# makezur/super_primitive

Hardware: AMD Instinct MI355X
Metric: GN iters/sec (640x480x64-seg frame pairs) (higher is better)
Workload: dtype f32; 1 GPU; Replica-shaped two-frame SfM, 640x480, 64 segments (grid, 4 px overlap), pyramid level 0 of a 3-level pyramid; BASELINE.json configs[1]; pairs_per_gpu=384, segment_pixels_per_pair=373056, optimiser=gn, tile_points=8192, span_points=4096, granule=64

## Files before the change

### super_primitive_amd/csrc/sp_cost.hip

```cpp
#include <type_traits>

#include "sp_solve_device.h"

namespace {

struct TileCtx {
    gptr_u32 pix;
    gptr_f4 src4;
    gptr_f32 trg;
    Cam Ks;
    Warp w;
    float shift;
    float gain, bias;
    float ax, ay;
    uint32_t row_bytes;
    int Wl, Hl;
    int start, count;
};

struct Geo {
    float qx, qy, qz;
    float zinv, zi;
    float px, py, pz;
};
// ... 194 lines not shown
    asm("v_pk_add_f32 %0, %1, %2 neg_lo:[0,1] neg_hi:[0,1]" : "=v"(d) : "v"(a), "v"(b));
    return d;
}
__device__ __forceinline__ f32x2 pmul_hi(f32x2 a, f32x2 b) {
    f32x2 d;
    asm("v_pk_mul_f32 %0, %1, %2 op_sel:[1,0] op_sel_hi:[1,1]" : "=v"(d) : "v"(a), "v"(b));
    return d;
}
__device__ __forceinline__ f32x2 pfma_lo(f32x2 a, f32x2 b, f32x2 c) {
    f32x2 d;
    asm("v_pk_fma_f32 %0, %1, %2, %3 op_sel:[0,0,0] op_sel_hi:[0,1,1]" : "=v"(d) : "v"(a), "v"(b), "v"(c));
    return d;
}
__device__ __forceinline__ f32x2 pfnma_lo(f32x2 a, f32x2 b, f32x2 c) {
    f32x2 d;
    asm("v_pk_fma_f32 %0, %1, %2, %3 op_sel:[0,0,0] op_sel_hi:[0,1,1] neg_lo:[1,0,0] neg_hi:[1,0,0]" : "=v"(d) : "v"(a), "v"(b), "v"(c));
    return d;
}
__device__ __forceinline__ f32x2 pfnma_hi(f32x2 a, f32x2 b, f32x2 c) {
    f32x2 d;
    asm("v_pk_fma_f32 %0, %1, %2, %3 op_sel:[1,0,0] op_sel_hi:[1,1,1] neg_lo:[1,0,0] neg_hi:[1,0,0]" : "=v"(d) : "v"(a), "v"(b), "v"(c));
    return d;
}
__device__ __forceinline__ f32x2 pfma_swz_lo(f32x2 a, f32x2 b, f32x2 c) {
    f32x2 d;
    asm("v_pk_fma_f32 %0, %1, %2, %3 op_sel:[1,0,0] op_sel_hi:[0,0,1]" : "=v"(d) : "v"(a), "v"(b), "v"(c));
    return d;
}
__device__ __forceinline__ f32x2 pfma_swz_hi(f32x2 a, f32x2 b, f32x2 c) {
    f32x2 d;
    asm("v_pk_fma_f32 %0, %1, %2, %3 op_sel:[1,1,0] op_sel_hi:[0,1,1]" : "=v"(d) : "v"(a), "v"(b), "v"(c));
    return d;
}
__device__ __forceinline__ f32x2 pmul_lo(f32x2 a, f32x2 b) {
    f32x2 d;
    asm("v_pk_mul_f32 %0, %1, %2 op_sel:[0,0] op_sel_hi:[0,1]" : "=v"(d) : "v"(a), "v"(b));
    return d;
}
__device__ __forceinline__ f32x2 pfma(float a, f32x2 b, f32x2 c) { return __builtin_elementwise_fma(f32x2{a, a}, b, c); }

struct GnAcc {
    f32x2 h00;
    f32x2 h0[2];
    f32x2 h1[2];
    f32x2 blk[6];
    f32x2 bp01;
    f32x2 bp[2];
    f32x2 hd01;
    f32x2 hd[2];
    float h11;
    f32x2 D, bd;
    float cost, n;
    float cost_mark, n_mark;
};

struct Pending2 {
    f32x2 qxy; float qz, zinv, zi;
    f32x2 wxy; float m;
    f32x2 srg; float sb;
    uint32_t off0;
};

__device__ __forceinline__ void prepare2_at(const PairConsts& k, f32x2 colrow, bool src_ok, float d, const f32x4 s, Pending2& p);

template <bool DT = false>
__device__ __forceinline__ void prepare2(const TileCtx& c, const PairConsts& k, float shift, uint32_t pw, const f32x4 s, Pending2& p) {
    const f32x2 colrow{(float)(pw & 0xffffu), (float)((pw >> 16) & 0x7fffu)};
    const bool src_ok = (int32_t)pw < 0;
    const float d = DT ? s.w * shift : fast_exp(s.w + shift);
    prepare2_at(k, colrow, src_ok, d, s, p);
}

typedef const SpRunDesc __attribute__((address_space(4)))* cptr_rd;
__device__ __forceinline__ SpRunDesc rd_load(cptr_rd p) {
    SpRunDesc r;
    r.valid[0] = p->valid[0]; r.valid[1] = p->valid[1];
    r.d[0] = p->d[0]; r.d[1] = p->d[1];
    r.base[0] = p->base[0]; r.base[1] = p->base[1];
    r.k = p->k; r.runs = p->runs;
    return r;
}
__device__ __forceinline__ f32x2 rd_colrow(const SpRunDesc& r, f32x2 lane2) {
    const float step = __builtin_amdgcn_fmed3f(lane2.x + r.k, 0.f, 1.f);
    return pfma(step, f32x2{r.d[0], r.d[1]}, lane2) + f32x2{r.base[0], r.base[1]};
}
__device__ __forceinline__ float rd_depth(const SpRunDesc& r, float d) {
    const uint64_t m = ((uint64_t)r.valid[1] << 32) | r.valid[0];
    float o;
    asm("v_cndmask_b32_e64 %0, 0, %1, %2" : "=v"(o) : "v"(d), "s"(m));
    return o;
}
template <bool DT>
__device__ __forceinline__ void prepare2_rd(const PairConsts& k, float shift, const SpRunDesc& r, f32x2 lane2, const f32x4 s, Pending2& p) {
    const f32x2 colrow = rd_colrow(r, lane2);
    const float d = rd_depth(r, DT ? s.w * shift : fast_exp(s.w + shift));
    prepare2_at(k, colrow, true, d, s, p);
}
template <bool DT>
__device__ __forceinline__ void prepare_rd(const TileCtx& c, float shift, float ifx, float ify, const SpRunDesc& r, f32x2 lane2, const f32x4 s,
                                           Pending& p) {
    const f32x2 colrow = rd_colrow(r, lane2);
    const float d = rd_depth(r, DT ? s.w * shift : fast_exp(s.w + shift));
    float x, y;
    backproject(colrow.x, colrow.y, d, c.Ks, ifx, ify, x, y);
    prepare_xyz(c, x, y, d, true, s.x, s.y, s.z, p);
}

__device__ __forceinline__ void prepare2_at(const PairConsts& k, f32x2 colrow, bool src_ok, float d, const f32x4 s, Pending2& p) {
    const f32x2 xy = pfma(colrow, k.ifxy, k.nKc) * d;
    const f32x2 qxy = pfma(k.R03, f32x2{xy.x, xy.x}, pfma(k.R14, f32x2{xy.y, xy.y}, pfma(k.R25, f32x2{d, d}, k.t01)));
    const float qz = fmaf(k.R6, xy.x, fmaf(k.R7, xy.y, fmaf(k.R8, d, k.t2)));
    const bool zguard = fabsf(qz) > 1e-6f;
    const float zinv = zguard ? __builtin_amdgcn_rcpf(qz) : 1e-6f;
    const f32x2 uv = qxy * k.Kf * zinv + k.Ktc;
    const f32x2 n = pfma(uv, k.invWH, f32x2{-1.f, -1.f});
    const bool ok = (fabsf(n.x) <= 0.99f) && (fabsf(n.y) <= 0.99f) && (qz > k.zmin) && src_ok && (d > 1e-7f);
    p.m = ok ? 1.f : 0.f;
    p.qxy = qxy; p.qz = qz;
    p.zinv = ok ? zinv : 0.f;
    p.zi = (ok && zguard) ? zinv : 0.f;
    p.srg = f32x2{s.x, s.y}; p.sb = s.z;
    const f32x2 ixy = pfma(n, k.sxy, k.sxy);
    const f32x2 fl{floorf(ixy.x), floorf(ixy.y)};
    p.wxy = ixy - fl;
    p.off0 = (uint32_t)fmaf(fl.y, k.row_bytes_f, fl.x * (float)(4u * SP_TEXEL_FLOATS));
}

struct Mix2 { f32x2 wa, wb, v; };
struct MixA { f32x2 ua, ub; };
struct AffAcc {
    float haa, hab, hbb, ba, bb;
    f32x2 pa01, pa[2], pb01, pb[2];
    float hda, hdb;
};

template <bool AFF = false>
__device__ __forceinline__ void finish_gn2(const PairConsts& k, const Pending2& p, const f32x3 a, const f32x3 b,
                                           const f32x3 cc, const f32x3 d, Mix2& o, float& cost_acc, float& n_acc,
                                           MixA* oa = nullptr, AffAcc* aa = nullptr) {
    const float eps = k.eps;
    const f32x2 a2{a.x, a.y}, b2{b.x, b.y}, c2{cc.x, cc.y}, d2{d.x, d.y};
    const f32x2 e3 = padd2(psub2(psub2(d2, c2), b2), a2);
    const f32x2 Er{b.x - a.x, cc.x - a.x}, Eg{b.y - a.y, cc.y - a.y}, Eb{b.z - a.z, cc.z - a.z};
    f32x2 e3b;
    e3b.x = (d.z - cc.z) - Eb.x;
    const f32x2 Gr = pfma_swz_lo(p.wxy, e3, Er), Gg = pfma_swz_hi(p.wxy, e3, Eg), Gb = pfma_swz_lo(p.wxy, e3b, Eb);
    const f32x2 it2{fmaf(p.wxy.y, Gr.y, fmaf(p.wxy.x, Er.x, a.x)), fmaf(p.wxy.y, Gg.y, fmaf(p.wxy.x, Eg.x, a.y))};
    const float itb = fmaf(p.wxy.y, Gb.y, fmaf(p.wxy.x, Eb.x, a.z));
    const f32x2 r2 = p.srg - pfma(k.gain, it2, k.bias2);
    const float rb = p.sb - fmaf(k.gain, itb, k.bias2.x);
    const float ar0 = fabsf(r2.x), ar1 = fabsf(r2.y), arb = fabsf(rb);
    auto absmax = [&](float r) { float m; asm("v_max_f32 %0, |%1|, %2" : "=v"(m) : "v"(r), "s"(eps)); return m; };
    const f32x2 wg2{__builtin_amdgcn_rcpf(absmax(r2.x)), __builtin_amdgcn_rcpf(absmax(r2.y))};
    const float wgb = __builtin_amdgcn_rcpf(absmax(rb));
    const f32x2 wGr = pmul_lo(wg2, Gr), wGg = pmul_hi(wg2, Gg), wGb = Gb * wgb;
    o.wa = pfma_lo(wGb, Gb, pfma_lo(wGg, Gg, pmul_lo(wGr, Gr)));
    o.wb = pfma_hi(wGb, Gb, pfma_hi(wGg, Gg, pmul_hi(wGr, Gr)));
    o.v = pfma(wGb, rb, pfma_hi(r2, wGg, pmul_lo(r2, wGr)));
    cost_acc = fmaf(p.m, (ar0 + ar1) + arb, cost_acc);
    n_acc += p.m;
    if constexpr (AFF) {
        const f32x2 ja2 = k.gain * it2;
        const float jab = k.gain * itb;
        const f32x2 wj2 = wg2 * ja2;
        const float wjb = wgb * jab;
        aa->haa = fmaf(p.m, fmaf(wjb, jab, wj2.x * ja2.x) + wj2.y * ja2.y, aa->haa);
        aa->hab = fmaf(-p.m, (wj2.x + wj2.y) + wjb, aa->hab);
        aa->hbb = fmaf(p.m, (wg2.x + wg2.y) + wgb, aa->hbb);
        aa->ba = fmaf(p.m, fmaf(wjb, rb, wj2.x * r2.x) + wj2.y * r2.y, aa->ba);
        aa->bb = fmaf(-p.m, fmaf(wgb, rb, wg2.x * r2.x) + wg2.y * r2.y, aa->bb);
        oa->ua = pfma(Gb, wjb, pfma_hi(wj2, Gg, pmul_lo(wj2, Gr)));
        oa->ub = (wGr + wGg) + wGb;
    }
}

struct GeoGn { f32x2 qxy; float qz, zinv, zi; };
template <bool AFF = false>
__device__ __forceinline__ void fold_gn2(const PairConsts& k, const GeoGn g, const Mix2 w, GnAcc& A, const MixA* wa = nullptr,
                                         AffAcc* aa = nullptr) {
    const f32x2 g2 = k.gab * g.zinv;
    const f32x2 Wa = w.wa * pmul_lo(g2, g2);
    const f32x2 Wb = w.wb * pmul_hi(g2, g2);
    const f32x2 V = -(w.v * g2);
    const f32x2 qxy = g.qxy;
    const f32x2 u = qxy * g.zi;
    const float ez = g.qz - k.t2;
    const f32x2 Q = pfma(-ez, u, qxy - k.t01);
    float nqy;
    asm("v_xor_b32 %0, 0x80000000, %1" : "=v"(nqy) : "v"(qxy.y));
    const f32x2 nA00{u.x, u.x * qxy.y}, A01{fmaf(u.x, qxy.x, g.qz), nqy};
    const f32x2 nA10{u.y, fmaf(u.y, qxy.y, g.qz)}, A11{u.y * qxy.x, qxy.x};
    const f32x2 nB00 = pfma_lo(Wa, nA00, pmul_hi(Wa, nA10)), B01 = pfma_lo(Wa, A01, pmul_hi(Wa, A11));
    const f32x2 nB10 = pfma_lo(Wb, nA00, pmul_hi(Wb, nA10)), B11 = pfma_lo(Wb, A01, pmul_hi(Wb, A11));
    const f32x2 P = pfma_lo(Q, Wa, pmul_hi(Q, Wb));
    A.h00 += Wa; A.h11 += Wb.y;
    A.h0[0] -= nB00; A.h0[1] += B01;
    A.h1[0] -= nB10; A.h1[1] += B11;
    A.blk[0] = pfma_lo(nA00, nB00, pfma_lo(nA10, nB10, A.blk[0]));
    A.blk[1] = pfnma_lo(nA00, B01, pfnma_lo(nA10, B11, A.blk[1]));
    A.blk[2] = pfma_hi(nA00, nB00, pfma_hi(nA10, nB10, A.blk[2]));
    A.blk[3] = pfnma_hi(nA00, B01, pfnma_hi(nA10, B11, A.blk[3]));
    A.blk[4] = pfma_lo(A01, B01, pfma_lo(A11, B11, A.blk[4]));
    A.blk[5] = pfma_hi(A01, B01, pfma_hi(A11, B11, A.blk[5]));
    A.bp01 += V;
    A.hd01 += P;
    A.bp[0] = pfnma_lo(V, nA00, pfnma_hi(V, nA10, A.bp[0]));
    A.bp[1] = pfma_lo(V, A01, pfma_hi(V, A11, A.bp[1]));
    A.hd[0] = pfnma_lo(P, nA00, pfnma_hi(P, nA10, A.hd[0]));
    A.hd[1] = pfma_lo(P, A01, pfma_hi(P, A11, A.hd[1]));
    A.D = pfma(Q, P, A.D);
    A.bd = pfma(Q, V, A.bd);
    if constexpr (AFF) {
        const f32x2 Ua = -(wa->ua * g2), Ub = wa->ub * g2;
        aa->pa01 += Ua;
        aa->pa[0] = pfnma_lo(Ua, nA00, pfnma_hi(Ua, nA10, aa->pa[0]));
        aa->pa[1] = pfma_lo(Ua, A01, pfma_hi(Ua, A11, aa->pa[1]));
        aa->hda = fmaf(Q.x, Ua.x, fmaf(Q.y, Ua.y, aa->hda));
        aa->pb01 += Ub;
        aa->pb[0] = pfnma_lo(Ub, nA00, pfnma_hi(Ub, nA10, aa->pb[0]));
        aa->pb[1] = pfma_lo(Ub, A01, pfma_hi(Ub, A11, aa->pb[1]));
        aa->hdb = fmaf(Q.x, Ub.x, fmaf(Q.y, Ub.y, aa->hdb));
    }
}

typedef const float __attribute__((address_space(4)))* cptr_f32;
struct ChunkRec { int pair, seg, start, count; };
typedef const ChunkRec __attribute__((address_space(4)))* cptr_i4;

struct SpanCursor {
    cptr_i4 chunks;
    cptr_f32 kld, kp_L;
    int q, q_end;
    int left;
    float shift;
    int nq_left;
    float nq_kld, nq_kpl;
};

template <int TRIP = SP_BLOCK>
__device__ __forceinline__ void cursor_fetch_next(SpanCursor& k) {
    if (k.q + 1 < k.q_end) {
        const int seg = k.chunks[k.q + 1].seg;
        k.nq_left = k.chunks[k.q + 1].count / TRIP;
        k.nq_kld = k.kld[seg];
        k.nq_kpl = k.kp_L[seg];
    }
}

template <bool DT>
__device__ __forceinline__ float cursor_shift(float kld, float kpl) { return DT ? fast_exp(kld - kpl) : kld - kpl; }

template <int TRIP = SP_BLOCK, bool DT = false>
__device__ __forceinline__ void cursor_init(SpanCursor& k, const SpPair& pr, const int4* chunks, int q0, int n) {
    k.chunks = (cptr_i4)chunks;
    k.kld = (cptr_f32)pr.kld;
    k.kp_L = (cptr_f32)pr.kp_L;
    k.q = q0; k.q_end = q0 + n;
    const int seg0 = k.chunks[q0].seg;
    k.left = k.chunks[q0].count / TRIP;
    k.shift = cursor_shift<DT>(k.kld[seg0], k.kp_L[seg0]);
    k.nq_left = 0; k.nq_kld = 0.f; k.nq_kpl = 0.f;
    cursor_fetch_next<TRIP>(k);
}

template <int TRIP = SP_BLOCK, bool DT = false>
__device__ __forceinline__ bool cursor_advance(SpanCursor& k, int& done_q) {
    done_q = k.q;
    if (--k.left > 0) return false;
    ++k.q;
    k.left = k.nq_left;
    k.shift = cursor_shift<DT>(k.nq_kld, k.nq_kpl);
    cursor_fetch_next<TRIP>(k);
    return true;
}

template <bool WT>
__device__ __forceinline__ void store_partial(float* p, float v) {
    if (WT) __hip_atomic_store(p, v, __ATOMIC_RELAXED, __HIP_MEMORY_SCOPE_AGENT);
    else *p = v;
}

__device__ __forceinline__ int lane_id() { return (int)__builtin_amdgcn_mbcnt_hi(~0u, __builtin_amdgcn_mbcnt_lo(~0u, 0u)); }

template <bool WT, bool AFF = false>
__device__ __forceinline__ void flush_segment_gn(GnAcc& A, float* __restrict__ rec, AffAcc* aa = nullptr) {
    const int lane = lane_id();
    int pos; bool ok;
    if constexpr (AFF) {
        float v[10] = {A.hd01.x, A.hd01.y, A.hd[0].x, A.hd[0].y, A.hd[1].x, A.hd[1].y, A.D.x + A.D.y, A.bd.x + A.bd.y, aa->hda, aa->hdb};
        wave_sum_to_lanes<10>(v, lane, pos, ok);
        if (ok) store_partial<WT>(rec + pos, v[0]);
        aa->hda = 0.f; aa->hdb = 0.f;
    } else {
        float v[10] = {A.hd01.x, A.hd01.y, A.hd[0].x, A.hd[0].y, A.hd[1].x, A.hd[1].y, A.D.x + A.D.y, A.bd.x + A.bd.y,
                       A.cost - A.cost_mark, A.n - A.n_mark};
        wave_sum_to_lanes<10>(v, lane, pos, ok);
        if (ok) store_partial<WT>(rec + pos, v[0]);
        A.cost_mark = A.cost; A.n_mark = A.n;
    }
    const f32x2 z{0.f, 0.f};
    A.hd01 = z; A.hd[0] = z; A.hd[1] = z; A.D = z; A.bd = z;
}

template <bool DT, bool WT, bool AFF = false, bool W64 = false, bool RD = false>
__device__ __forceinline__ void run_span_gn(const TileCtx& c, const SpPair& pr, const int4* __restrict__ chunks, int q0,
                                            int n_chunks, int total, float irls_eps, float* __restrict__ span_rec,
                                            float* __restrict__ seg_partials, float* lds, const SpRunDesc* rd = nullptr) {
    static_assert(!RD || (W64 && DT && !AFF), "run descriptors: wave spans on depth tables");
    constexpr int TRIP = W64 ? 64 : SP_BLOCK;
    constexpr int NV = AFF ? SP_GNA_PARTIAL_FLOATS : SP_GN_PARTIAL_FLOATS, NS = AFF ? SP_GNA_SEG_FLOATS : SP_GN_SEG_FLOATS;
    GnAcc A;
    AffAcc AA;
    MixA ma{f32x2{0.f, 0.f}, f32x2{0.f, 0.f}};
    {
        const f32x2 z{0.f, 0.f};
        AA.haa = AA.hab = AA.hbb = AA.ba = AA.bb = AA.hda = AA.hdb = 0.f;
        AA.pa01 = z; AA.pb01 = z; AA.pa[0] = z; AA.pa[1] = z; AA.pb[0] = z; AA.pb[1] = z;
    }
    {
        const f32x2 z{0.f, 0.f};
        A.h00 = z; A.bp01 = z; A.hd01 = z;
#pragma unroll
        for (int k = 0; k < 2; ++k) { A.h0[k] = z; A.h1[k] = z; A.bp[k] = z; A.hd[k] = z; }
#pragma unroll
        for (int k = 0; k < 6; ++k) A.blk[k] = z;
        A.D = z; A.bd = z;
        A.h11 = A.cost = A.n = A.cost_mark = A.n_mark = 0.f;
    }
    const int wave = __builtin_amdgcn_readfirstlane((int)(threadIdx.x >> 6));
    SpanCursor k;
    cursor_init<TRIP, DT>(k, pr, chunks, q0, n_chunks);
    const int start = k.chunks[q0].start;
    PairConsts kc;
    {
        const Warp& w = c.w;
        kc.ifxy = sgpr2(1.f / c.Ks.fx, 1.f / c.Ks.fy);
        kc.nKc = f32x2{-c.Ks.cx * (1.f / c.Ks.fx), -c.Ks.cy * (1.f / c.Ks.fy)};
        kc.R03 = sgpr2(w.R[0], w.R[3]);        kc.R14 = sgpr2(w.R[1], w.R[4]);      kc.R25 = sgpr2(w.R[2], w.R[5]);
        kc.t01 = f32x2{w.t[0], w.t[1]};        kc.Kf = sgpr2(w.Kt.fx, w.Kt.fy);     kc.Ktc = sgpr2(w.Kt.cx, w.Kt.cy);
        kc.invWH = sgpr2(2.f * w.invWm1, 2.f * w.invHm1);  kc.sxy = sgpr2(w.sx, w.sy);
        kc.gab = sgpr2(c.gain * c.ax * w.Kt.fx, c.gain * c.ay * w.Kt.fy);
        kc.bias2 = f32x2{c.bias, c.bias};      kc.eps2 = sgpr2(irls_eps, irls_eps);
        kc.R6 = sgpr(w.R[6]); kc.R7 = sgpr(w.R[7]); kc.R8 = sgpr(w.R[8]); kc.t2 = w.t[2];
        asm volatile("" : "+v"(kc.nKc), "+v"(kc.bias2), "+v"(kc.t01), "+v"(kc.t2));
        kc.gain = sgpr(c.gain); kc.bias = sgpr(c.bias); kc.zmin = sgpr(w.zmin); kc.eps = sgpr(irls_eps);
        kc.row_bytes_f = sgpr((float)(c.Wl * (int)(4u * SP_TEXEL_FLOATS)));
    }
    const rsrc_t r_pix = make_rsrc(c.pix + start, (uint32_t)total * 4u);
    const rsrc_t r_src = make_rsrc(c.src4 + start, (uint32_t)total * 16u);
    const rsrc_t r_trg = make_rsrc(c.trg, (uint32_t)c.Wl * (uint32_t)c.Hl * (4u * SP_TEXEL_FLOATS));
    const int n_iter = total / TRIP;
    uint32_t op = (W64 ? (threadIdx.x & 63u) : threadIdx.x) * 4u;
    constexpr int NT = 2;
    cptr_rd rg = (cptr_rd)rd + (start >> 6);
    f32x2 lane2{(float)(threadIdx.x & 63u), 0.f};
    if (RD) asm volatile("" : "+v"(lane2));
    struct Slot { Pending2 p; int q; bool last; };
    Slot S0, S1;
    {
        const f32x4 s = buf_load4<NT>(r_src, op * 4u);
        if (RD) prepare2_rd<DT>(kc, k.shift, rd_load(rg), lane2, s, S0.p);
        else {
            const uint32_t pw = (uint32_t)__builtin_amdgcn_raw_buffer_load_b32(r_pix, (int)op, 0, NT);
            prepare2<DT>(c, kc, k.shift, pw, s, S0.p);
        }
        S0.last = cursor_advance<TRIP, DT>(k, S0.q);
    }
    S1.p = S0.p;
    S1.p.zinv = 0.f; S1.p.zi = 0.f;
    S1.q = q0; S1.last = false;
    Mix2 m{f32x2{0.f, 0.f}, f32x2{0.f, 0.f}, f32x2{0.f, 0.f}};
    auto trip = [&](Slot& a, Slot& b) {
        op += 4u * TRIP;
        asm volatile("" : "+v"(op));
        const uint32_t pw = RD ? 0u : (uint32_t)__builtin_amdgcn_raw_buffer_load_b32(r_pix, (int)op, 0, NT);
        const f32x4 s = buf_load4<NT>(r_src, op * 4u);
        SpRunDesc rn;
        if (RD) { ++rg; rn = rd_load(rg); }
        f32x3 ta = buf_load3(r_trg, a.p.off0);
        f32x3 tb = buf_load3(r_trg, a.p.off0 + 4u * SP_TEXEL_FLOATS);
        f32x3 tc = buf_load3(r_trg, a.p.off0, c.row_bytes);
        f32x3 td = buf_load3(r_trg, a.p.off0 + 4u * SP_TEXEL_FLOATS, c.row_bytes);
        __builtin_amdgcn_sched_barrier(0);
        fold_gn2<AFF>(kc, GeoGn{b.p.qxy, b.p.qz, b.p.zinv, b.p.zi}, m, A, &ma, &AA);
        if (b.last) flush_segment_gn<WT, AFF>(A, seg_partials + (size_t)(W64 ? b.q : 4 * b.q + wave) * NS, &AA);
        __builtin_amdgcn_sched_barrier(0);
        asm volatile("" : "+v"(ta), "+v"(tb), "+v"(tc), "+v"(td), "+v"(A.blk[0]), "+v"(A.blk[1]), "+v"(A.blk[2]),
                     "+v"(A.blk[3]), "+v"(A.blk[4]), "+v"(A.blk[5]), "+v"(A.bp[0]), "+v"(A.bp[1]), "+v"(A.hd[0]),
                     "+v"(A.hd[1]), "+v"(A.D), "+v"(A.bd), "+v"(A.h00), "+v"(A.h0[0]), "+v"(A.h0[1]), "+v"(A.h1[0]), "+v"(A.h1[1]), "+v"(A.h11), "+v"(A.bp01), "+v"(A.hd01));
        finish_gn2<AFF>(kc, a.p, ta, tb, tc, td, m, A.cost, A.n, &ma, &AA);
        uint32_t pw_ = pw;
        f32x4 s_ = s;
        if (RD) asm volatile("" : "+v"(s_));
        else asm volatile("" : "+v"(pw_), "+v"(s_));
        if (RD) prepare2_rd<DT>(kc, k.shift, rn, lane2, s_, b.p);
        else prepare2<DT>(c, kc, k.shift, pw_, s_, b.p);
        b.last = cursor_advance<TRIP, DT>(k, b.q);
    };
    int j = 0;
    for (; j + 1 < n_iter; j += 2) { trip(S0, S1); trip(S1, S0); }
    if (j < n_iter) {
        trip(S0, S1);
        fold_gn2<AFF>(kc, GeoGn{S0.p.qxy, S0.p.qz, S0.p.zinv, S0.p.zi}, m, A, &ma, &AA);
        flush_segment_gn<WT, AFF>(A, seg_partials + (size_t)(W64 ? S0.q : 4 * S0.q + wave) * NS, &AA);
    } else {
        fold_gn2<AFF>(kc, GeoGn{S1.p.qxy, S1.p.qz, S1.p.zinv, S1.p.zi}, m, A, &ma, &AA);
        flush_segment_gn<WT, AFF>(A, seg_partials + (size_t)(W64 ? S1.q : 4 * S1.q + wave) * NS, &AA);
    }
    float acc[NV];
    acc[0] = A.cost;
    acc[1] = A.h00.x; acc[2] = A.h00.y;
    acc[3] = A.h0[0].x; acc[4] = A.h0[0].y; acc[5] = A.h0[1].x; acc[6] = A.h0[1].y;
    acc[7] = A.h11;
    acc[8] = A.h1[0].x; acc[9] = A.h1[0].y; acc[10] = A.h1[1].x; acc[11] = A.h1[1].y;
    acc[12] = A.blk[0].x; acc[13] = A.blk[0].y; acc[14] = A.blk[1].x; acc[15] = A.blk[1].y;
    acc[16] = A.blk[2].y; acc[17] = A.blk[3].x; acc[18] = A.blk[3].y;
    acc[19] = A.blk[4].x; acc[20] = A.blk[4].y; acc[21] = A.blk[5].y;
    acc[22] = A.bp01.x; acc[23] = A.bp01.y;
    acc[24] = A.bp[0].x; acc[25] = A.bp[0].y; acc[26] = A.bp[1].x; acc[27] = A.bp[1].y;
    acc[28] = A.n;
    if constexpr (AFF) {
        acc[29] = AA.haa; acc[30] = AA.hab; acc[31] = AA.hbb; acc[32] = AA.ba; acc[33] = AA.bb;
        acc[34] = AA.pa01.x; acc[35] = AA.pa01.y; acc[36] = AA.pa[0].x; acc[37] = AA.pa[0].y; acc[38] = AA.pa[1].x; acc[39] = AA.pa[1].y;
        acc[40] = AA.pb01.x; acc[41] = AA.pb01.y; acc[42] = AA.pb[0].x; acc[43] = AA.pb[0].y; acc[44] = AA.pb[1].x; acc[45] = AA.pb[1].y;
        acc[46] = acc[47] = 0.f;
    } else {
        acc[29] = acc[30] = acc[31] = 0.f;
    }
    if (W64) {
        int pos; bool ok;
        wave_sum_to_lanes<NV>(acc, (int)((op >> 2) & 63u), pos, ok);
        if (ok) store_partial<WT>(span_rec + pos, acc[0]);
    } else {
        const int tid = (int)((op >> 2) & (uint32_t)(SP_BLOCK - 1));
        const float tot = block_sum_to_thread<NV>(acc, lds, tid);
        if (tid < NV) store_partial<WT>(span_rec + tid, tot);
    }
}

template <bool DT, bool WT, bool W64 = false, bool RD = false>
__device__ __forceinline__ void run_span_grad(const TileCtx& c, const SpPair& pr, const int4* __restrict__ chunks, int q0,
                                              int n_chunks, int total, float* __restrict__ span_rec,
                                              float* __restrict__ seg_partials, float* lds, const SpRunDesc* rd = nullptr) {
    static_assert(!RD || (W64 && DT), "run descriptors: wave spans on depth tables");
    constexpr int TRIP = W64 ? 64 : SP_BLOCK;
    constexpr int NV = SP_GRAD_PARTIAL_FLOATS;
    float acc[NV];
#pragma unroll
    for (int i = 0; i < NV; ++i) acc[i] = 0.f;
    const int wave = __builtin_amdgcn_readfirstlane((int)(threadIdx.x >> 6));
    SpanCursor k;
    cursor_init<TRIP, DT>(k, pr, chunks, q0, n_chunks);
    const int start = k.chunks[q0].start;
    const float ifx = 1.f / c.Ks.fx, ify = 1.f / c.Ks.fy;
    const rsrc_t r_pix = make_rsrc(c.pix + start, (uint32_t)total * 4u);
    const rsrc_t r_src = make_rsrc(c.src4 + start, (uint32_t)total * 16u);
    const rsrc_t r_trg = make_rsrc(c.trg, (uint32_t)c.Wl * (uint32_t)c.Hl * (4u * SP_TEXEL_FLOATS));
    const int n_iter = total / TRIP;
    uint32_t op = (W64 ? (threadIdx.x & 63u) : threadIdx.x) * 4u;
    constexpr int NT = 2;
    cptr_rd rg = (cptr_rd)rd + (start >> 6);
    f32x2 lane2{(float)(threadIdx.x & 63u), 0.f};
    if (RD) asm volatile("" : "+v"(lane2));
    struct Slot { Pending p; int q; bool last; };
    Slot S0, S1;
    {
        const f32x4 s = buf_load4<NT>(r_src, op * 4u);
        if (RD) prepare_rd<DT>(c, k.shift, ifx, ify, rd_load(rg), lane2, s, S0.p);
        else {
            const uint32_t pw = (uint32_t)__builtin_amdgcn_raw_buffer_load_b32(r_pix, (int)op, 0, NT);
            prepare<DT>(c, k.shift, ifx, ify, pw, s, S0.p);
        }
        S0.last = cursor_advance<TRIP, DT>(k, S0.q);
    }
    S1.p = S0.p;
    S1.p.g.zinv = 0.f; S1.p.g.zi = 0.f;
    S1.q = q0; S1.last = false;
    Mix0 m0{0.f, 0.f, 0.f, 0.f};
    auto flush = [&](int q) {
        const float tot = wave_sum(acc[13]);
        if (lane_id() == 0) store_partial<WT>(seg_partials + (size_t)(W64 ? q : 4 * q + wave) * SP_GRAD_SEG_FLOATS, tot);
        acc[13] = 0.f;
    };
    auto trip = [&](Slot& a, Slot& b) {
        op += 4u * TRIP;
        asm volatile("" : "+v"(op));
        const uint32_t pw = RD ? 0u : (uint32_t)__builtin_amdgcn_raw_buffer_load_b32(r_pix, (int)op, 0, NT);
        const f32x4 s = buf_load4<NT>(r_src, op * 4u);
        SpRunDesc rn;
        if (RD) { ++rg; rn = rd_load(rg); }
        f32x3 ta = buf_load3(r_trg, a.p.off0);
        f32x3 tb = buf_load3(r_trg, a.p.off0 + 4u * SP_TEXEL_FLOATS);
        f32x3 tc = buf_load3(r_trg, a.p.off0, c.row_bytes);
        f32x3 td = buf_load3(r_trg, a.p.off0 + 4u * SP_TEXEL_FLOATS, c.row_bytes);
        __builtin_amdgcn_sched_barrier(0);
        fold_grad(c, b.p.g, m0, acc);
        if (b.last) flush(b.q);
        __builtin_amdgcn_sched_barrier(0);
        asm volatile("" : "+v"(ta), "+v"(tb), "+v"(tc), "+v"(td), "+v"(acc[1]), "+v"(acc[2]), "+v"(acc[3]), "+v"(acc[4]), "+v"(acc[5]),
                     "+v"(acc[6]), "+v"(acc[7]), "+v"(acc[8]), "+v"(acc[9]), "+v"(acc[10]), "+v"(acc[11]), "+v"(acc[12]),
                     "+v"(acc[13]), "+v"(acc[14]), "+v"(acc[15]));
        finish_grad(c, a.p, ta, tb, tc, td, m0, acc[0]);
        uint32_t pw_ = pw;
        f32x4 s_ = s;
        if (RD) asm volatile("" : "+v"(s_));
        else asm volatile("" : "+v"(pw_), "+v"(s_));
        if (RD) prepare_rd<DT>(c, k.shift, ifx, ify, rn, lane2, s_, b.p);
        else prepare<DT>(c, k.shift, ifx, ify, pw_, s_, b.p);
        b.last = cursor_advance<TRIP, DT>(k, b.q);
    };
    int j = 0;
    for (; j + 1 < n_iter; j += 2) { trip(S0, S1); trip(S1, S0); }
    if (j < n_iter) {
        trip(S0, S1);
        fold_grad(c, S0.p.g, m0, acc);
        flush(S0.q);
    } else {
        fold_grad(c, S1.p.g, m0, acc);
        flush(S1.q);
    }
    if (W64) {
        int pos; bool ok;
        wave_sum_to_lanes<NV>(acc, (int)((op >> 2) & 63u), pos, ok);
        if (ok) store_partial<WT>(span_rec + pos, acc[0]);
    } else {
        const int tid = (int)((op >> 2) & (uint32_t)(SP_BLOCK - 1));
        const float tot = block_sum_to_thread<NV>(acc, lds, tid);
        if (tid < NV) store_partial<WT>(span_rec + tid, tot);
    }
}

__device__ __forceinline__ void fill_warp(TileCtx& c, const float* pose, const Cam& Kt, int H, int W, int Hl, int Wl,
                                          float zmin) {
    load_pose(pose, c.w.R, c.w.t);
    c.w.Kt = Kt;
    c.w.invWm1 = sgpr(1.f / (float)(W - 1));
    c.w.invHm1 = sgpr(1.f / (float)(H - 1));
    c.w.sx = sgpr(0.5f * (float)(Wl - 1));
    c.w.sy = sgpr(0.5f * (float)(Hl - 1));
    c.w.zmin = zmin;
    c.Wl = Wl; c.Hl = Hl;
    c.row_bytes = (uint32_t)Wl * (4u * SP_TEXEL_FLOATS);
    c.ax = sgpr(2.f * c.w.sx * c.w.invWm1);
    c.ay = sgpr(2.f * c.w.sy * c.w.invHm1);
}


struct SingleArgs {
    const uint32_t* pix; const float4* src4; const float* kp_L; const int4* tiles;
    const float* K_src; const float* kld; const float* trg; const float* K_trg; const float* pose;
    const float* aff_src; const float* aff_trg;
    int n_tiles, H, W, Hl, Wl;
    float zmin;
};

__global__ __launch_bounds__(SP_BLOCK) void k_cost_single_grad(SingleArgs a, float* __restrict__ partials) {
    __shared__ float lds[SP_WAVES * SP_GRAD_PARTIAL_FLOATS];
    const int t = xcd_chunked_tile(blockIdx.x, a.n_tiles);
    if (t >= a.n_tiles) return;
    const int b = blockIdx.y;
    const int4 tile = a.tiles[t];
    TileCtx c;
    c.pix = (gptr_u32)a.pix; c.src4 = (gptr_f4)a.src4;
    c.trg = (gptr_f32)(a.trg + (size_t)b * a.Hl * a.Wl * SP_TEXEL_FLOATS);
    load_cam(a.K_src, c.Ks);
    Cam Kt; load_cam(a.K_trg + 9 * b, Kt);
    fill_warp(c, a.pose + 16 * b, Kt, a.H, a.W, a.Hl, a.Wl, a.zmin);
    c.shift = a.kld[tile.y] - a.kp_L[tile.y];
    c.gain = 1.f; c.bias = 0.f;
    if (a.aff_src) {
        c.gain = expf(-(a.aff_trg[2 * b] - a.aff_src[0]));
        c.bias = a.aff_trg[2 * b + 1] - a.aff_src[1];
    }
    c.start = tile.z; c.count = tile.w;
    run_tile<false>(c, partials + ((size_t)b * a.n_tiles + t) * SP_GRAD_PARTIAL_FLOATS, lds);
}

#define SP_POINT_TILE 2048
struct PointsArgs {
    const float* xyz; const float* rgb; const float* trg; const float* K_trg; const float* pose;
    const float* aff_src; const float* aff_trg;
    int n_points, n_tiles, H, W, Hl, Wl;
    float zmin;
};

__global__ __launch_bounds__(SP_BLOCK) void k_cost_points_grad(PointsArgs a, float* __restrict__ partials) {
    __shared__ float lds[SP_WAVES * SP_GRAD_PARTIAL_FLOATS];
    const int t = xcd_chunked_tile(blockIdx.x, a.n_tiles);
    if (t >= a.n_tiles) return;
    const int b = blockIdx.y;
    TileCtx c;
    c.pix = (gptr_u32)a.xyz; c.src4 = (gptr_f4)a.rgb;
    c.trg = (gptr_f32)(a.trg + (size_t)b * a.Hl * a.Wl * SP_TEXEL_FLOATS);
    c.Ks = Cam{1.f, 1.f, 0.f, 0.f};
    Cam Kt; load_cam(a.K_trg + 9 * b, Kt);
    fill_warp(c, a.pose + 16 * b, Kt, a.H, a.W, a.Hl, a.Wl, a.zmin);
    c.shift = 0.f;
    c.gain = 1.f; c.bias = 0.f;
    if (a.aff_src) {
        c.gain = expf(-(a.aff_trg[2 * b] - a.aff_src[0]));
        c.bias = a.aff_trg[2 * b + 1] - a.aff_src[1];
    }
    c.start = t * SP_POINT_TILE;
    c.count = min(SP_POINT_TILE, a.n_points - c.start);
    run_tile<true>(c, partials + ((size_t)b * a.n_tiles + t) * SP_GRAD_PARTIAL_FLOATS, lds);
}

__global__ __launch_bounds__(SP_BLOCK) void k_finalise_single(const float* __restrict__ partials,
                                                               const int32_t* __restrict__ seg_tile_off, int n_tiles,
                                                               int N, int P, bool has_aff, float* residual,
                                                               float* g_kld, float* g_pose, float* g_aff) {
    const int b = blockIdx.x;
    const float* p = partials + (size_t)b * n_tiles * SP_GRAD_PARTIAL_FLOATS;
    const double scale = 1.0 / (3.0 * (double)P);
    const int lane = threadIdx.x & 63, wave = threadIdx.x >> 6;
    for (int k = wave; k < SP_GRAD_PARTIAL_FLOATS; k += SP_WAVES) {
        if (k == 13) continue;
        double s = 0.0;
        for (int t = lane; t < n_tiles; t += 64) s += (double)p[(size_t)t * SP_GRAD_PARTIAL_FLOATS + k];
#pragma unroll
        for (int o = 32; o > 0; o >>= 1) s += __shfl_xor(s, o, 64);
        if (lane == 0) {
            const float v = (float)(s * scale);
            if (k == 0) residual[b] = v;
            else if (k <= 3) g_pose[b * 16 + (k - 1) * 4 + 3] = v;
            else if (k <= 12) { const int e = k - 4; g_pose[b * 16 + (e / 3) * 4 + (e % 3)] = v; }
            else if (k == 14) { g_aff[b * 4 + 2] = has_aff ? v : 0.f; g_aff[b * 4 + 0] = has_aff ? -v : 0.f; }
            else { g_aff[b * 4 + 3] = has_aff ? v : 0.f; g_aff[b * 4 + 1] = has_aff ? -v : 0.f; }
        }
    }
    if (threadIdx.x < 4) g_pose[b * 16 + 12 + threadIdx.x] = 0.f;
    for (int n = threadIdx.x; n < N; n += SP_BLOCK) {
        double s = 0.0;
        for (int t = seg_tile_off[n]; t < seg_tile_off[n + 1]; ++t) s += (double)p[(size_t)t * SP_GRAD_PARTIAL_FLOATS + 13];
        g_kld[(size_t)b * N + n] = (float)(s * scale);
    }
}

#define SP_SCHED_LISTS 8
struct SchedList {
    const int4* chunks;
    const int4* spans;
    float* partials;
    float* seg_partials;
    int32_t n_spans;
    int32_t first_block;
    uint32_t mask;
    int32_t vspans;
};
struct SchedCost {
    const SpPair* pairs[SP_MAX_PHASES];
    float irls_eps[SP_MAX_PHASES];
    uint32_t mask;
    int32_t vspans;
    int32_t n_lists;
    SchedList list[SP_SCHED_LISTS];
};
struct FuseArgs {
    int32_t* arrivals;
    AdamArgs adam;
    GnArgs gn;
    const int32_t* done;
    const int32_t* phase;
    SchedCost sched;
    const int32_t* active;
    const MultiList* multi;
    int32_t n_multi;
    const uint32_t* rd_pix;
    const SpRunDesc* rd_desc;
};

constexpr int FORM_LOG_DEPTH = 0, FORM_DEPTH = 6;

struct Pix;
struct RunDesc;
template <class SRC>
struct CostFrom {
template <int MODE, int FORM = FORM_LOG_DEPTH, int FUSED = 0, bool W64 = false>
static __global__ __launch_bounds__(SP_BLOCK, FUSED != 0 ? 1 : (MODE == 2 ? 2 : 4)) void k_cost_pairs(
        const SpPair* __restrict__ pairs, const int4* __restrict__ chunks, const int4* __restrict__ spans, int n_spans,
        float irls_eps, float* __restrict__ partials, float* __restrict__ seg_partials, FuseArgs f) {
    static_assert(FORM == FORM_LOG_DEPTH || FORM == FORM_DEPTH, "FORM: log-depth tables (0) or depth tables (6)");
    constexpr bool RD = std::is_same<SRC, RunDesc>::value;
    constexpr bool DT = FORM == FORM_DEPTH;
    constexpr int NV = MODE == 0 ? SP_GRAD_PARTIAL_FLOATS : (MODE == 2 ? SP_GNA_PARTIAL_FLOATS : SP_GN_PARTIAL_FLOATS);
    __shared__ float lds[SP_WAVES * NV];
    int block = blockIdx.x;
    uint32_t phase_mask = f.sched.mask;
    int vspans = f.sched.vspans;
    if (f.multi) {
        int l = 0;
        for (int i = 1; i < f.n_multi && block >= f.multi[i].first_block; ++i) l = i;
        const MultiList& ml = f.multi[l];
        block -= ml.first_block;
        pairs = ml.pairs; chunks = reinterpret_cast<const int4*>(ml.chunks); spans = reinterpret_cast<const int4*>(ml.spans);
        n_spans = ml.n_spans; partials = ml.partials; seg_partials = ml.seg_partials;
    }
    if (f.phase && f.sched.n_lists > 0) {
        int l = 0;
#pragma unroll
        for (int i = 1; i < SP_SCHED_LISTS; ++i)
            if (i < f.sched.n_lists && block >= f.sched.list[i].first_block) l = i;
        const SchedList& sl = f.sched.list[l];
        block -= sl.first_block;
        chunks = sl.chunks; spans = sl.spans; n_spans = sl.n_spans; partials = sl.partials; seg_partials = sl.seg_partials;
        phase_mask = sl.mask;
        vspans = sl.vspans;
    }
    int w = W64 ? 4 * xcd_chunked_tile(block, (n_spans + 3) >> 2) + __builtin_amdgcn_readfirstlane((int)(threadIdx.x >> 6))
                : xcd_chunked_tile(block, n_spans);
    if (w >= n_spans) return;
    int owner;
    int4 span;
    if (MODE == 1 && FUSED == 0 && f.phase && vspans > 0) {
        owner = w / vspans;
        const int j = w - owner * vspans;
        if (f.active) owner = f.active[owner];
        const int ph = f.phase[owner];
        if (ph >= SP_MAX_PHASES || ph < 0 || !((phase_mask >> ph) & 1u)) return;
        pairs = f.sched.pairs[ph];
        irls_eps = f.sched.irls_eps[ph];
        if (j >= pairs[owner].n_tiles) return;
        w = pairs[owner].tile0 + j;
        span = spans[w];
    } else {
        span = spans[w];
        owner = span.w;
        if (f.done && f.done[owner]) return;
        if (f.phase) {
            const int ph = f.phase[owner];
            if (ph >= SP_MAX_PHASES || ph < 0 || !((phase_mask >> ph) & 1u)) return;
            pairs = f.sched.pairs[ph];
            irls_eps = f.sched.irls_eps[ph];
        }
    }
    const SpPair& pr = pairs[owner];
    TileCtx c;
    c.pix = (gptr_u32)pr.pix;
    c.src4 = (gptr_f4)pr.src4;
    c.trg = (gptr_f32)pr.trg3;
    c.Ks = Cam{pr.K_src[0], pr.K_src[1], pr.K_src[2], pr.K_src[3]};
    const Cam Kt{pr.K_trg[0], pr.K_trg[1], pr.K_trg[2], pr.K_trg[3]};
    fill_warp(c, pr.pose, Kt, pr.H, pr.W, pr.Hl, pr.Wl, pr.zmin);
    c.shift = 0.f;
    c.gain = 1.f; c.bias = 0.f;
    if (pr.aff) {
        c.gain = sgpr(expf(-(pr.aff[2] - pr.aff[0])));
        c.bias = sgpr(pr.aff[3] - pr.aff[1]);
    }
    c.start = 0; c.count = 0;
    const SpRunDesc* rd = RD ? f.rd_desc + ((const uint32_t*)pr.pix - f.rd_pix) / 64 : nullptr;
    if (MODE == 2) run_span_gn<DT, FUSED != 0, true>(c, pr, chunks, span.x, span.y, span.z, irls_eps, partials + (size_t)w * NV, seg_partials, lds);
    else if (MODE == 1) run_span_gn<DT, FUSED != 0, false, W64, RD>(c, pr, chunks, span.x, span.y, span.z, irls_eps, partials + (size_t)w * NV, seg_partials, lds, rd);
    else run_span_grad<DT, FUSED != 0, W64, RD>(c, pr, chunks, span.x, span.y, span.z, partials + (size_t)w * NV, seg_partials, lds, rd);
    if (FUSED != 0) {
        __shared__ int is_last;
        asm volatile("s_waitcnt vmcnt(0)" ::: "memory");
        __syncthreads();
        if (threadIdx.x == 0) {
            const int old = __hip_atomic_fetch_add(f.arrivals + span.w, 1, __ATOMIC_RELAXED, __HIP_MEMORY_SCOPE_AGENT);
            const int last = old == pr.n_tiles - 1;
            if (last) {
                __hip_atomic_store(f.arrivals + span.w, 0, __ATOMIC_RELAXED, __HIP_MEMORY_SCOPE_AGENT);
                __builtin_amdgcn_fence(__ATOMIC_ACQUIRE, "agent");
            }
            is_last = last;
        }
        __syncthreads();
        if (is_last) {
            if (FUSED == 1) solve_adam(pairs, span.w, partials, seg_partials, f.adam);
            else solve_gn(pairs, span.w, partials, seg_partials, f.gn);
        }
    }
}
};

struct CostVariant {
    int mode;
    bool dt, w64, rd;
    int fused;
};
using CostKernel = void (*)(const SpPair*, const int4*, const int4*, int, float, float*, float*, FuseArgs);
CostKernel cost_kernel(const CostVariant& v) {
    enum { DT = 4, W64 = 8, RD = 16, ADAM = 32, GN = 2 * ADAM };
    if (v.mode < 0 || v.mode > 2 || v.fused < 0 || v.fused > 2) return nullptr;
    switch (v.mode | (v.dt ? DT : 0) | (v.w64 ? W64 : 0) | (v.rd ? RD : 0) | v.fused * ADAM) {
        case 0:                 return CostFrom<Pix>::k_cost_pairs<0>;
        case 1:                 return CostFrom<Pix>::k_cost_pairs<1>;
        case 2:                 return CostFrom<Pix>::k_cost_pairs<2>;
        case 0 | DT:            return CostFrom<Pix>::k_cost_pairs<0, FORM_DEPTH>;
        case 1 | DT:            return CostFrom<Pix>::k_cost_pairs<1, FORM_DEPTH>;
        case 0 | W64:           return CostFrom<Pix>::k_cost_pairs<0, FORM_LOG_DEPTH, 0, true>;
        case 1 | W64:           return CostFrom<Pix>::k_cost_pairs<1, FORM_LOG_DEPTH, 0, true>;
        case 0 | DT | W64:      return CostFrom<Pix>::k_cost_pairs<0, FORM_DEPTH, 0, true>;
        case 1 | DT | W64:      return CostFrom<Pix>::k_cost_pairs<1, FORM_DEPTH, 0, true>;
        case 0 | DT | W64 | RD: return CostFrom<RunDesc>::k_cost_pairs<0, FORM_DEPTH, 0, true>;
        case 1 | DT | W64 | RD: return CostFrom<RunDesc>::k_cost_pairs<1, FORM_DEPTH, 0, true>;
        case 0 | ADAM:          return CostFrom<Pix>::k_cost_pairs<0, FORM_LOG_DEPTH, 1>;
        case 1 | GN:            return CostFrom<Pix>::k_cost_pairs<1, FORM_LOG_DEPTH, 2>;
        default:                return nullptr;
    }
}

int cost_blocks(int n_spans, bool w64) { return (((w64 ? (n_spans + 3) / 4 : n_spans) + 7) / 8) * 8; }

int launch_cost(const CostVariant& v, int blocks, hipStream_t s, const SpPair* pairs, const int32_t* chunks, const int32_t* spans, int n_spans,
                float irls_eps, float* partials, float* seg_partials, const FuseArgs& f) {
    const CostKernel k = cost_kernel(v);
    if (!k) return SP_EINVAL;
    const int4* c4 = reinterpret_cast<const int4*>(chunks);
    const int4* s4 = reinterpret_cast<const int4*>(spans);
    hipLaunchKernelGGL(k, dim3(blocks), dim3(SP_BLOCK), 0, s, pairs, c4, s4, n_spans, irls_eps, partials, seg_partials, f);
    SP_CHECK_LAUNCH();
    return 0;
}

struct StatsArgs {
    const uint32_t* pix; const float4* src4; const int32_t* seg_off; const float* kp_L;
    const float* K_src; const float* kld; const float* trg; const float* K_trg; const float* pose;
    const float* aff_src; const float* aff_trg;
    int N, P, H, W, Hl, Wl;
    int stride, Pout;
    float zmin;
// ... 267 lines not shown
```

Baseline: 435,700 iters/s.

## Prefetch source pixel and colour streams two trips ahead in span loops

Deepens the software pipeline in the GN and gradient span loops so the pixel-index and source-colour buffer loads are issued one extra trip earlier. The stream buffer descriptors are offset by one trip, so the loads land in alternating StreamRec registers. Colour values are copied into fresh registers so the prefetch destinations can be overwritten sooner. The aim is to hide streaming load latency behind the gather and fold arithmetic, at the cost of extra VGPRs that could reduce occupancy.

```diff
diff --git a/super_primitive_amd/csrc/sp_cost.hip b/super_primitive_amd/csrc/sp_cost.hip
--- a/super_primitive_amd/csrc/sp_cost.hip
+++ b/super_primitive_amd/csrc/sp_cost.hip
@@ -520,6 +520,20 @@
     A.hd01 = z; A.hd[0] = z; A.hd[1] = z; A.D = z; A.bd = z;
 }
 
+constexpr int SP_STREAM_AHEAD_GN = 2;
+constexpr int SP_STREAM_AHEAD_GNA = 2;
+constexpr int SP_STREAM_AHEAD_GRAD = 2;
+struct StreamRec { f32x4 s; uint32_t pw; };
+__device__ __forceinline__ void detach_colour(f32x2& rg, float& b) {
+    asm("v_mov_b64 %0, %1" : "=v"(rg) : "v"(rg));
+    asm("v_mov_b32 %0, %1" : "=v"(b) : "v"(b));
+}
+__device__ __forceinline__ void detach_colour(float& r, float& g, float& b) {
+    asm("v_mov_b32 %0, %1" : "=v"(r) : "v"(r));
+    asm("v_mov_b32 %0, %1" : "=v"(g) : "v"(g));
+    asm("v_mov_b32 %0, %1" : "=v"(b) : "v"(b));
+}
+
 template <bool DT, bool WT, bool AFF = false, bool W64 = false, bool RD = false>
 __device__ __forceinline__ void run_span_gn(const TileCtx& c, const SpPair& pr, const int4* __restrict__ chunks, int q0,
                                             int n_chunks, int total, float irls_eps, float* __restrict__ span_rec,
@@ -564,8 +578,11 @@
         kc.gain = sgpr(c.gain); kc.bias = sgpr(c.bias); kc.zmin = sgpr(w.zmin); kc.eps = sgpr(irls_eps);
         kc.row_bytes_f = sgpr((float)(c.Wl * (int)(4u * SP_TEXEL_FLOATS)));
     }
-    const rsrc_t r_pix = make_rsrc(c.pix + start, (uint32_t)total * 4u);
-    const rsrc_t r_src = make_rsrc(c.src4 + start, (uint32_t)total * 16u);
+    constexpr int AHEAD = AFF ? SP_STREAM_AHEAD_GNA : SP_STREAM_AHEAD_GN;
+    constexpr int SKIP = (AHEAD - 1) * TRIP;
+    const uint32_t n_ahead = SKIP ? (uint32_t)max(total - SKIP, 0) : (uint32_t)total;
+    const rsrc_t r_pix = make_rsrc(c.pix + start + SKIP, n_ahead * 4u);
+    const rsrc_t r_src = make_rsrc(c.src4 + start + SKIP, n_ahead * 16u);
     const rsrc_t r_trg = make_rsrc(c.trg, (uint32_t)c.Wl * (uint32_t)c.Hl * (4u * SP_TEXEL_FLOATS));
     const int n_iter = total / TRIP;
     uint32_t op = (W64 ? (threadIdx.x & 63u) : threadIdx.x) * 4u;
@@ -575,30 +592,37 @@
     if (RD) asm volatile("" : "+v"(lane2));
     struct Slot { Pending2 p; int q; bool last; };
     Slot S0, S1;
+    StreamRec R0, R1;
+    auto stream = [&](StreamRec& r) {
+        r.pw = RD ? 0u : (uint32_t)__builtin_amdgcn_raw_buffer_load_b32(r_pix, (int)op, 0, NT);
+        r.s = buf_load4<NT>(r_src, op * 4u);
+    };
     {
-        const f32x4 s = buf_load4<NT>(r_src, op * 4u);
+        const f32x4 s = buf_load4<NT>(make_rsrc(c.src4 + start, (uint32_t)total * 16u), op * 4u);
+        const uint32_t pw = RD ? 0u : (uint32_t)__builtin_amdgcn_raw_buffer_load_b32(make_rsrc(c.pix + start, (uint32_t)total * 4u), (int)op, 0, NT);
+        if (AHEAD == 2) stream(R1);
         if (RD) prepare2_rd<DT>(kc, k.shift, rd_load(rg), lane2, s, S0.p);
-        else {
-            const uint32_t pw = (uint32_t)__builtin_amdgcn_raw_buffer_load_b32(r_pix, (int)op, 0, NT);
-            prepare2<DT>(c, kc, k.shift, pw, s, S0.p);
-        }
+        else prepare2<DT>(c, kc, k.shift, pw, s, S0.p);
         S0.last = cursor_advance<TRIP, DT>(k, S0.q);
     }
     S1.p = S0.p;
     S1.p.zinv = 0.f; S1.p.zi = 0.f;
     S1.q = q0; S1.last = false;
     Mix2 m{f32x2{0.f, 0.f}, f32x2{0.f, 0.f}, f32x2{0.f, 0.f}};
-    auto trip = [&](Slot& a, Slot& b) {
+    auto trip = [&](Slot& a, Slot& b, StreamRec& ld, StreamRec& use) {
         op += 4u * TRIP;
         asm volatile("" : "+v"(op));
-        const uint32_t pw = RD ? 0u : (uint32_t)__builtin_amdgcn_raw_buffer_load_b32(r_pix, (int)op, 0, NT);
-        const f32x4 s = buf_load4<NT>(r_src, op * 4u);
+        if (AHEAD == 1) stream(ld);
         SpRunDesc rn;
         if (RD) { ++rg; rn = rd_load(rg); }
         f32x3 ta = buf_load3(r_trg, a.p.off0);
         f32x3 tb = buf_load3(r_trg, a.p.off0 + 4u * SP_TEXEL_FLOATS);
         f32x3 tc = buf_load3(r_trg, a.p.off0, c.row_bytes);
         f32x3 td = buf_load3(r_trg, a.p.off0 + 4u * SP_TEXEL_FLOATS, c.row_bytes);
+        if (AHEAD == 2) {
+            __builtin_amdgcn_sched_barrier(0);
+            stream(ld);
+        }
         __builtin_amdgcn_sched_barrier(0);
         fold_gn2<AFF>(kc, GeoGn{b.p.qxy, b.p.qz, b.p.zinv, b.p.zi}, m, A, &ma, &AA);
         if (b.last) flush_segment_gn<WT, AFF>(A, seg_partials + (size_t)(W64 ? b.q : 4 * b.q + wave) * NS, &AA);
@@ -607,24 +631,27 @@
                      "+v"(A.blk[3]), "+v"(A.blk[4]), "+v"(A.blk[5]), "+v"(A.bp[0]), "+v"(A.bp[1]), "+v"(A.hd[0]),
                      "+v"(A.hd[1]), "+v"(A.D), "+v"(A.bd), "+v"(A.h00), "+v"(A.h0[0]), "+v"(A.h0[1]), "+v"(A.h1[0]), "+v"(A.h1[1]), "+v"(A.h11), "+v"(A.bp01), "+v"(A.hd01));
         finish_gn2<AFF>(kc, a.p, ta, tb, tc, td, m, A.cost, A.n, &ma, &AA);
-        uint32_t pw_ = pw;
-        f32x4 s_ = s;
+        uint32_t pw_ = use.pw;
+        f32x4 s_ = use.s;
         if (RD) asm volatile("" : "+v"(s_));
         else asm volatile("" : "+v"(pw_), "+v"(s_));
         if (RD) prepare2_rd<DT>(kc, k.shift, rn, lane2, s_, b.p);
         else prepare2<DT>(c, kc, k.shift, pw_, s_, b.p);
+        if (AHEAD == 2) detach_colour(b.p.srg, b.p.sb);
+        if (AHEAD == 2 && !RD) asm volatile("" : "+v"(b.p.m));
         b.last = cursor_advance<TRIP, DT>(k, b.q);
     };
+    auto last = [&](Slot& f) {
+        fold_gn2<AFF>(kc, GeoGn{f.p.qxy, f.p.qz, f.p.zinv, f.p.zi}, m, A, &ma, &AA);
+        flush_segment_gn<WT, AFF>(A, seg_partials + (size_t)(W64 ? f.q : 4 * f.q + wave) * NS, &AA);
+    };
+    StreamRec& RB = AHEAD == 2 ? R1 : R0;
     int j = 0;
-    for (; j + 1 < n_iter; j += 2) { trip(S0, S1); trip(S1, S0); }
+    for (; j + 1 < n_iter; j += 2) { trip(S0, S1, R0, RB); trip(S1, S0, RB, R0); }
     if (j < n_iter) {
-        trip(S0, S1);
-        fold_gn2<AFF>(kc, GeoGn{S0.p.qxy, S0.p.qz, S0.p.zinv, S0.p.zi}, m, A, &ma, &AA);
-        flush_segment_gn<WT, AFF>(A, seg_partials + (size_t)(W64 ? S0.q : 4 * S0.q + wave) * NS, &AA);
-    } else {
-        fold_gn2<AFF>(kc, GeoGn{S1.p.qxy, S1.p.qz, S1.p.zinv, S1.p.zi}, m, A, &ma, &AA);
-        flush_segment_gn<WT, AFF>(A, seg_partials + (size_t)(W64 ? S1.q : 4 * S1.q + wave) * NS, &AA);
-    }
+        trip(S0, S1, R0, RB);
+        last(S0);
+    } else last(S1);
     float acc[NV];
     acc[0] = A.cost;
     acc[1] = A.h00.x; acc[2] = A.h00.y;
@@ -671,8 +698,11 @@
     cursor_init<TRIP, DT>(k, pr, chunks, q0, n_chunks);
     const int start = k.chunks[q0].start;
     const float ifx = 1.f / c.Ks.fx, ify = 1.f / c.Ks.fy;
-    const rsrc_t r_pix = make_rsrc(c.pix + start, (uint32_t)total * 4u);
-    const rsrc_t r_src = make_rsrc(c.src4 + start, (uint32_t)total * 16u);
+    constexpr int AHEAD = SP_STREAM_AHEAD_GRAD;
+    constexpr int SKIP = (AHEAD - 1) * TRIP;
+    const uint32_t n_ahead = SKIP ? (uint32_t)max(total - SKIP, 0) : (uint32_t)total;
+    const rsrc_t r_pix = make_rsrc(c.pix + start + SKIP, n_ahead * 4u);
+    const rsrc_t r_src = make_rsrc(c.src4 + start + SKIP, n_ahead * 16u);
     const rsrc_t r_trg = make_rsrc(c.trg, (uint32_t)c.Wl * (uint32_t)c.Hl * (4u * SP_TEXEL_FLOATS));
     const int n_iter = total / TRIP;
     uint32_t op = (W64 ? (threadIdx.x & 63u) : threadIdx.x) * 4u;
@@ -682,13 +712,17 @@
     if (RD) asm volatile("" : "+v"(lane2));
     struct Slot { Pending p; int q; bool last; };
     Slot S0, S1;
+    StreamRec R0, R1;
+    auto stream = [&](StreamRec& r) {
+        r.pw = RD ? 0u : (uint32_t)__builtin_amdgcn_raw_buffer_load_b32(r_pix, (int)op, 0, NT);
+        r.s = buf_load4<NT>(r_src, op * 4u);
+    };
     {
-        const f32x4 s = buf_load4<NT>(r_src, op * 4u);
+        const f32x4 s = buf_load4<NT>(make_rsrc(c.src4 + start, (uint32_t)total * 16u), op * 4u);
+        const uint32_t pw = RD ? 0u : (uint32_t)__builtin_amdgcn_raw_buffer_load_b32(make_rsrc(c.pix + start, (uint32_t)total * 4u), (int)op, 0, NT);
+        if (AHEAD == 2) stream(R1);
         if (RD) prepare_rd<DT>(c, k.shift, ifx, ify, rd_load(rg), lane2, s, S0.p);
-        else {
-            const uint32_t pw = (uint32_t)__builtin_amdgcn_raw_buffer_load_b32(r_pix, (int)op, 0, NT);
-            prepare<DT>(c, k.shift, ifx, ify, pw, s, S0.p);
-        }
+        else prepare<DT>(c, k.shift, ifx, ify, pw, s, S0.p);
         S0.last = cursor_advance<TRIP, DT>(k, S0.q);
     }
     S1.p = S0.p;
@@ -700,17 +734,20 @@
         if (lane_id() == 0) store_partial<WT>(seg_partials + (size_t)(W64 ? q : 4 * q + wave) * SP_GRAD_SEG_FLOATS, tot);
         acc[13] = 0.f;
     };
-    auto trip = [&](Slot& a, Slot& b) {
+    auto trip = [&](Slot& a, Slot& b, StreamRec& ld, StreamRec& use) {
         op += 4u * TRIP;
         asm volatile("" : "+v"(op));
-        const uint32_t pw = RD ? 0u : (uint32_t)__builtin_amdgcn_raw_buffer_load_b32(r_pix, (int)op, 0, NT);
-        const f32x4 s = buf_load4<NT>(r_src, op * 4u);
+        if (AHEAD == 1) stream(ld);
         SpRunDesc rn;
         if (RD) { ++rg; rn = rd_load(rg); }
         f32x3 ta = buf_load3(r_trg, a.p.off0);
         f32x3 tb = buf_load3(r_trg, a.p.off0 + 4u * SP_TEXEL_FLOATS);
         f32x3 tc = buf_load3(r_trg, a.p.off0, c.row_bytes);
         f32x3 td = buf_load3(r_trg, a.p.off0 + 4u * SP_TEXEL_FLOATS, c.row_bytes);
+        if (AHEAD == 2) {
+            __builtin_amdgcn_sched_barrier(0);
+            stream(ld);
+        }
         __builtin_amdgcn_sched_barrier(0);
         fold_grad(c, b.p.g, m0, acc);
         if (b.last) flush(b.q);
@@ -719,24 +756,26 @@
                      "+v"(acc[6]), "+v"(acc[7]), "+v"(acc[8]), "+v"(acc[9]), "+v"(acc[10]), "+v"(acc[11]), "+v"(acc[12]),
                      "+v"(acc[13]), "+v"(acc[14]), "+v"(acc[15]));
         finish_grad(c, a.p, ta, tb, tc, td, m0, acc[0]);
-        uint32_t pw_ = pw;
-        f32x4 s_ = s;
+        uint32_t pw_ = use.pw;
+        f32x4 s_ = use.s;
         if (RD) asm volatile("" : "+v"(s_));
         else asm volatile("" : "+v"(pw_), "+v"(s_));
         if (RD) prepare_rd<DT>(c, k.shift, ifx, ify, rn, lane2, s_, b.p);
         else prepare<DT>(c, k.shift, ifx, ify, pw_, s_, b.p);
+        if (AHEAD == 2) detach_colour(b.p.sr, b.p.sg, b.p.sb);
         b.last = cursor_advance<TRIP, DT>(k, b.q);
     };
+    auto last = [&](Slot& f) {
+        fold_grad(c, f.p.g, m0, acc);
+        flush(f.q);
+    };
+    StreamRec& RB = AHEAD == 2 ? R1 : R0;
     int j = 0;
-    for (; j + 1 < n_iter; j += 2) { trip(S0, S1); trip(S1, S0); }
+    for (; j + 1 < n_iter; j += 2) { trip(S0, S1, R0, RB); trip(S1, S0, RB, R0); }
     if (j < n_iter) {
-        trip(S0, S1);
-        fold_grad(c, S0.p.g, m0, acc);
-        flush(S0.q);
-    } else {
-        fold_grad(c, S1.p.g, m0, acc);
-        flush(S1.q);
-    }
+        trip(S0, S1, R0, RB);
+        last(S0);
+    } else last(S1);
     if (W64) {
         int pos; bool ok;
         wave_sum_to_lanes<NV>(acc, (int)((op >> 2) & 63u), pos, ok);
```

After: 435,900 iters/s, median of 2. Within noise of the previous version (+0.0%).
